# tangjiapeng/DiffuScene

Hardware: AMD Instinct MI355X
Metric: denoiser steps/sec (train + 1000-step sample) at B=256, N=80 objects (higher is better)
Workload: dtype f32 (operands split 3xbf16, 6 products, f32 accumulate); 1 GPU; uncond living/dining rooms (config/uncond/diffusion_livingrooms_instancond_lat32_v.yaml scaled to N=80), B=256 scenes per GPU, N=80, C=65, T=1000, mode=both; global_batch=256, parallelism=single

## Files before the change

### diffuscene_amd/_lib.py

```python
import ctypes as C
import os

_HERE = os.path.dirname(os.path.abspath(__file__))
LIB_PATH = os.path.join(_HERE, "libdiffuscene_hip.so")
if os.environ.get("DSC_HIP_LIB"):
    LIB_PATH = os.path.abspath(os.environ["DSC_HIP_LIB"])

ACT_NONE, ACT_GELU, ACT_SILU, ACT_LEAKY01 = 0, 1, 2, 3
SS_NONE, SS_PER_TOKEN, SS_PER_SCENE, SS_PER_SLOT, SS_BY_INDEX = 0, 1, 2, 3, 4
MEAN_EPS, MEAN_X0, MEAN_V = 0, 1, 2
TILE_GN_80_W8, TILE_GN_80_W4, TILE_160x256, TILE_160x128_W4 = 1, 2, 5, 8
TILE_WAVE_GN, TILE_WAVE_DENSE, TILE_WAVE_GN_64 = 10, 11, 12
F32_TILE_160x256, F32_TILE_160x128, F32_TILE_128x128, F32_TILE_96x128, F32_TILE_64x64 = 0, 1, 2, 3, 4
DSC_PLANES_NONE = -100
GEMM_ROW_INVARIANT = 1
WS_MAX = 64
MAX_TOKENS_PER_SCENE = 160
STATS_MAX_OBJECTS, STATS_ONE_WAVE_MAX = 160, 32

_ERR = {-1: "DSC_EINVAL (bad shape / null pointer)", -2: "DSC_EALIGN (16-byte alignment required)",
        -3: "DSC_ERANGE (size outside kernel limits)"}

c_f32p = C.c_void_p
c_i64p = C.c_void_p
# ... 63 lines not shown

class ColsumItem(C.Structure):
    _fields_ = [("x", C.c_void_p), ("ldx", C.c_int64), ("m", C.c_int32), ("n", C.c_int32), ("out", C.c_void_p)]


class WsBwdItem(C.Structure):
    _fields_ = [("w", C.c_void_p), ("dw_std", C.c_void_p), ("dw", C.c_void_p), ("rows", C.c_int32), ("cols", C.c_int32)]


SIGNATURES = {
    "dsc_version": (C.c_int, []),
    "dsc_gemm_f32": (C.c_int, [C.POINTER(GemmArgs), C.c_void_p]),
    "dsc_gemm_gn_silu_f32": (C.c_int, [C.POINTER(GemmArgs), C.c_void_p]),
    "dsc_split_bf16x3_f32": (C.c_int, [C.POINTER(SplitItem), C.c_int32, C.c_void_p]),
    "dsc_gemm_arithmetic": (C.c_int, [C.POINTER(GemmArgs), C.c_int32]),
    "dsc_gemm_split_tile": (C.c_int, [C.POINTER(GemmArgs), C.c_int32]),
    "dsc_gemm_f32_tile": (C.c_int, [C.POINTER(GemmArgs)]),
    "dsc_gemm_planes_layout": (C.c_int, [C.POINTER(GemmArgs), C.c_int32]),
    "dsc_get_split_wave": (C.c_int, []),
    "dsc_set_split_wave": (C.c_int, [C.c_int32]),
    "dsc_gemm_skinny": (C.c_int, [C.POINTER(GemmArgs), C.c_int32]),
    "dsc_get_skinny": (C.c_int, []),
    "dsc_set_skinny": (C.c_int, [C.c_int32]),
    "dsc_get_gemm_arithmetic": (C.c_int, []),
    "dsc_set_gemm_arithmetic": (C.c_int, [C.c_int32]),
    "dsc_gemm_layernorm_f32": (C.c_int, [C.POINTER(GemmArgs), C.c_void_p]),
    "dsc_gemm_splitk_f32": (C.c_int, [C.POINTER(GemmArgs), C.c_int32, c_f32p, C.c_int64, C.c_void_p]),
    "dsc_linear_smallk_f32": (C.c_int, [c_f32p, C.c_int64, C.c_int32, c_f32p, C.c_int64, c_f32p, c_f32p, C.c_int64,
                                        C.c_int32, C.c_int32, C.c_int32, C.c_void_p]),
    "dsc_linear_smallk_grouped_f32": (C.c_int, [C.POINTER(SmallKItem), C.c_int32, C.c_int32, C.c_int32, C.c_int32, C.c_void_p]),
    "dsc_gather_columns_f32": (C.c_int, [c_f32p, C.c_int64, c_f32p, C.c_int64, C.c_int32, C.POINTER(ColSpan), C.c_int32, C.c_void_p]),
    "dsc_weight_standardize_f32": (C.c_int, [C.POINTER(WsItem), C.c_int32, C.c_float, C.c_void_p]),
    "dsc_layernorm_f32": (C.c_int, [c_f32p, C.c_int64, c_f32p, c_f32p, C.c_int64, c_f32p, C.c_int64, C.c_int32,
                                    C.c_int32, C.c_float, C.c_void_p]),
    "dsc_linear_attention_f32": (C.c_int, [c_f32p, C.c_int64, c_f32p, C.c_int64, c_f32p, C.c_int64, c_f32p, C.c_int64,
                                           C.c_int32, C.c_int32, C.c_int32, C.c_float, C.c_void_p]),
    "dsc_attention_f32": (C.c_int, [c_f32p, C.c_int64, c_f32p, C.c_int64, c_f32p, C.c_int64, c_f32p, C.c_int64,
                                    C.c_int32, C.c_int32, C.c_float, C.c_void_p]),
    "dsc_time_embedding_f32": (C.c_int, [c_i64p, C.c_int32, C.c_int32, c_f32p, C.c_int32, c_f32p, c_f32p, C.c_void_p]),
    "dsc_activation_f32": (C.c_int, [c_f32p, c_f32p, C.c_int64, C.c_int32, C.c_void_p]),
    "dsc_q_sample_f32": (C.c_int, [c_f32p, c_f32p, c_i64p, c_f32p, c_f32p, c_f32p, c_f32p, C.c_int32, C.c_int64, C.c_int32,
                                   C.c_void_p]),
    "dsc_p_sample_f32": (C.c_int, [c_f32p, c_f32p, c_f32p, c_i64p, c_f32p, c_f32p, c_f32p, c_f32p, c_f32p, c_f32p,
                                   c_f32p, C.c_int32, C.c_int32, C.c_int32, C.c_int64, C.c_int32, C.c_void_p]),
    "dsc_device_error_count": (C.c_int64, [C.c_int32]),
    "dsc_add_scalar_i64": (C.c_int, [c_i64p, C.c_int32, C.c_int64, C.c_void_p]),
# ... 174 lines not shown
```

### diffuscene_amd/csrc/blocks.hip

```cpp
#include "dsc_common.h"

namespace {

struct WsBatch { dsc_ws_item it[DSC_WS_MAX]; };

__device__ __forceinline__ float block_sum_256(float v, float* red) {
    v = wave_sum(v);
    const int lane = threadIdx.x & 63, wave = threadIdx.x >> 6;
    __syncthreads();
    if (lane == 0) red[wave] = v;
    __syncthreads();
    return red[0] + red[1] + red[2] + red[3];
}

__global__ __launch_bounds__(256) void ws_kernel(const WsBatch b, const float eps) {
    __shared__ float red[4];
    const dsc_ws_item it = b.it[blockIdx.y];
    const int row = blockIdx.x;
    if (row >= it.rows) return;
    const float* w = it.w + (int64_t)row * it.cols;
    float* o = it.out + (int64_t)row * it.cols;
    constexpr int MAXE = 8;
    float v[MAXE];
    float s = 0.f;
// ... 40 lines not shown
    }
    const float var = wave_sum(s2) * (1.0f / 512.0f);
    const float rs = 1.0f / sqrtf(var + eps);
    const f32x4 ga = *reinterpret_cast<const f32x4*>(g + lane * 4);
    const f32x4 gb = *reinterpret_cast<const f32x4*>(g + 256 + lane * 4);
    f32x4 oa, ob;
#pragma unroll
    for (int e = 0; e < 4; ++e) {
        oa[e] = (a[e] - mean) * rs * ga[e];
        ob[e] = (b[e] - mean) * rs * gb[e];
    }
    if (res) {
        const float* rr = res + (int64_t)row * ldr;
        const f32x4 ra = *reinterpret_cast<const f32x4*>(rr + lane * 4);
        const f32x4 rb = *reinterpret_cast<const f32x4*>(rr + 256 + lane * 4);
#pragma unroll
        for (int e = 0; e < 4; ++e) { oa[e] += ra[e]; ob[e] += rb[e]; }
    }
    float* yr = y + (int64_t)row * ldy;
    *reinterpret_cast<f32x4*>(yr + lane * 4) = oa;
    *reinterpret_cast<f32x4*>(yr + 256 + lane * 4) = ob;
}

constexpr int MAXTOK = 160;
constexpr int HP = 33;
constexpr int LP = 36;

__global__ __launch_bounds__(256) void linear_attention_kernel(const float* __restrict__ q, int64_t ldq,
                                                               const float* __restrict__ k, int64_t ldk,
                                                               const float* __restrict__ v, int64_t ldv,
                                                               float* __restrict__ out, int64_t ldo,
                                                               int nq, int nk, float scale) {
    extern __shared__ __attribute__((aligned(16))) float lds[];
    float* Ks = lds;
    float* Vs = Ks + nk * LP;
    float* Qs = Vs + nk * LP;
    float* ctx = Qs + nq * LP;
    const int b = blockIdx.x >> 2, h = blockIdx.x & 3;
    const int tid = threadIdx.x;
    const float* kb = k + (int64_t)b * nk * ldk + h * 32;
    const float* vb = v + (int64_t)b * nk * ldv + h * 32;
    const float* qb = q + (int64_t)b * nq * ldq + h * 32;
    for (int f = tid; f < nk * 8; f += 256) {
        const int j = f >> 3, c4 = (f & 7) * 4;
        *reinterpret_cast<f32x4*>(Ks + j * LP + c4) = *reinterpret_cast<const f32x4*>(kb + (int64_t)j * ldk + c4);
        *reinterpret_cast<f32x4*>(Vs + j * LP + c4) = *reinterpret_cast<const f32x4*>(vb + (int64_t)j * ldv + c4);
    }
    for (int f = tid; f < nq * 8; f += 256) {
        const int i = f >> 3, c4 = (f & 7) * 4;
// ... 60 lines not shown
#pragma unroll
            for (int e = 0; e < 4; ++e) { a[e] = qv[e] * inv; c[e] = qv[4 + e] * inv; }
            *reinterpret_cast<f32x4*>(Qs + i * LP + part * 8) = a;
            *reinterpret_cast<f32x4*>(Qs + i * LP + part * 8 + 4) = c;
        }
        __builtin_amdgcn_wave_barrier();
        if (ok) {
            f32x4 o0 = {0.f, 0.f, 0.f, 0.f}, o1 = {0.f, 0.f, 0.f, 0.f};
#pragma unroll 8
            for (int d = 0; d < 32; ++d) {
                const float qd = Qs[i * LP + d];
                const f32x4 c0 = *reinterpret_cast<const f32x4*>(ctx + d * LP + part * 8);
                const f32x4 c1 = *reinterpret_cast<const f32x4*>(ctx + d * LP + part * 8 + 4);
#pragma unroll
                for (int e = 0; e < 4; ++e) { o0[e] += c0[e] * qd; o1[e] += c1[e] * qd; }
            }
            float* orow = out + ((int64_t)b * nq + i) * ldo + h * 32 + part * 8;
            *reinterpret_cast<f32x4*>(orow) = o0;
            *reinterpret_cast<f32x4*>(orow + 4) = o1;
        }
    }
}

__global__ __launch_bounds__(512) void attention_kernel(const float* __restrict__ q, int64_t ldq,
                                                        const float* __restrict__ k, int64_t ldk,
                                                        const float* __restrict__ v, int64_t ldv,
                                                        float* __restrict__ out, int64_t ldo, int n, float scale) {
    extern __shared__ __attribute__((aligned(16))) float att_lds[];
    float* Ks = att_lds;
    float* Vs = Ks + n * LP;
    const int b = blockIdx.x >> 2, h = blockIdx.x & 3;
    const int tid = threadIdx.x;
    const float* kb = k + (int64_t)b * n * ldk + h * 32;
    const float* vb = v + (int64_t)b * n * ldv + h * 32;
    const int nthr = blockDim.x, rows = nthr >> 2;
    for (int f = tid; f < n * 8; f += nthr) {
        const int j = f >> 3, c4 = (f & 7) * 4;
        *reinterpret_cast<f32x4*>(Ks + j * LP + c4) = *reinterpret_cast<const f32x4*>(kb + (int64_t)j * ldk + c4);
        *reinterpret_cast<f32x4*>(Vs + j * LP + c4) = *reinterpret_cast<const f32x4*>(vb + (int64_t)j * ldv + c4);
    }
    __syncthreads();
    const int part = tid & 3;
    for (int i0 = 0; i0 < n; i0 += rows) {
        const int i = i0 + (tid >> 2);
        const bool ok = i < n;
        const float* qr = q + ((int64_t)b * n + (ok ? i : 0)) * ldq + h * 32 + part * 8;
// ... 147 lines not shown
        if (items[i].cols > 2048) return DSC_ERANGE;
        b.it[i] = items[i];
        if (items[i].rows > maxrows) maxrows = items[i].rows;
    }
    DSC_CLEAR_STALE_ERROR();
    hipLaunchKernelGGL(ws_kernel, dim3(maxrows, count), dim3(256), 0, static_cast<hipStream_t>(stream), b, eps);
    DSC_LAUNCH_CHECK();
    return 0;
}

extern "C" int dsc_layernorm_f32(const float* x, int64_t ldx, const float* g, const float* residual, int64_t ldr,
                                 float* y, int64_t ldy, int32_t m, int32_t d, float eps, dsc_stream_t stream) {
    if (!x || !g || !y || m < 1) return DSC_EINVAL;
    if (d != 512) return DSC_ERANGE;
    if (!dsc_aligned16(x) || !dsc_aligned16(g) || !dsc_aligned16(y) || (ldx & 3) || (ldy & 3)) return DSC_EALIGN;
    if (residual && (!dsc_aligned16(residual) || (ldr & 3))) return DSC_EALIGN;
    DSC_CLEAR_STALE_ERROR();
    hipLaunchKernelGGL(layernorm512_kernel, dim3((m + 3) / 4), dim3(256), 0, static_cast<hipStream_t>(stream),
                       x, ldx, g, residual, ldr, y, ldy, m, eps);
    DSC_LAUNCH_CHECK();
    return 0;
}

extern "C" int dsc_linear_attention_f32(const float* q, int64_t ldq, const float* k, int64_t ldk,
                                        const float* v, int64_t ldv, float* out, int64_t ldo,
                                        int32_t scenes, int32_t nq, int32_t nk, float scale, dsc_stream_t stream) {
    if (!q || !k || !v || !out || scenes < 1 || nq < 1 || nk < 1) return DSC_EINVAL;
    if (nk > MAXTOK) return DSC_ERANGE;
    if (!dsc_aligned16(q) || !dsc_aligned16(k) || !dsc_aligned16(v) || !dsc_aligned16(out) ||
        (ldq & 3) || (ldk & 3) || (ldv & 3) || (ldo & 3)) return DSC_EALIGN;
    if (nq > MAXTOK) return DSC_ERANGE;
    const size_t lds = sizeof(float) * ((size_t)(2 * nk + nq) * LP + 32 * LP);
    static bool attr_set = false;
    if (!attr_set) {
        hipError_t e = hipFuncSetAttribute(reinterpret_cast<const void*>(linear_attention_kernel),
                                           hipFuncAttributeMaxDynamicSharedMemorySize, 96 * 1024);
        if (e != hipSuccess) return (int)e;
        attr_set = true;
    }
    DSC_CLEAR_STALE_ERROR();
    hipLaunchKernelGGL(linear_attention_kernel, dim3(scenes * DSC_HEADS), dim3(256), lds,
                       static_cast<hipStream_t>(stream), q, ldq, k, ldk, v, ldv, out, ldo, nq, nk, scale);
    DSC_LAUNCH_CHECK();
    return 0;
}

extern "C" int dsc_attention_f32(const float* q, int64_t ldq, const float* k, int64_t ldk,
                                 const float* v, int64_t ldv, float* out, int64_t ldo,
                                 int32_t scenes, int32_t n, float scale, dsc_stream_t stream) {
    if (!q || !k || !v || !out || scenes < 1 || n < 1) return DSC_EINVAL;
    if (n > MAXTOK) return DSC_ERANGE;
    if (!dsc_aligned16(q) || !dsc_aligned16(k) || !dsc_aligned16(v) || !dsc_aligned16(out) ||
        (ldq & 3) || (ldk & 3) || (ldv & 3) || (ldo & 3)) return DSC_EALIGN;
    DSC_CLEAR_STALE_ERROR();
// ... 75 lines not shown
```

### diffuscene_amd/csrc/dsc_common.h

```cpp
#pragma once
#include <hip/hip_runtime.h>
#include <stdint.h>
#include <type_traits>
#include "../../include/diffuscene_hip.h"

typedef float f32x2 __attribute__((ext_vector_type(2)));
typedef float f32x4 __attribute__((ext_vector_type(4)));
typedef float f32x16 __attribute__((ext_vector_type(16)));

#define DSC_WAVE 64

#include <utility>
template <class F, int... I>
__device__ __forceinline__ void dsc_static_for_impl(F&& f, std::integer_sequence<int, I...>) { (f(std::integral_constant<int, I>{}), ...); }
template <int N, class F>
__device__ __forceinline__ void dsc_static_for(F&& f) { dsc_static_for_impl(f, std::make_integer_sequence<int, N>{}); }

#define DSC_CLEAR_STALE_ERROR() ((void)hipGetLastError())

#define DSC_LAUNCH_CHECK()                                   \
    do {                                                     \
        hipError_t e__ = hipGetLastError();                  \
        if (e__ != hipSuccess) return (int)e__;              \
    } while (0)
// ... 25 lines not shown
        const float t = __builtin_amdgcn_rcpf(fmaf(0.3275911f, a, 1.0f));
        float p = fmaf(1.061405429f, t, -1.453152027f);
        p = fmaf(p, t, 1.421413741f);
        p = fmaf(p, t, -0.284496736f);
        p = fmaf(p, t, 0.254829592f);
        const float e = __expf(-a * a);
        const float cdf = 0.5f * (1.0f + copysignf(1.0f - p * t * e, xv));
        return fmaf(xv * 0.39894228040143267794f, e, cdf);
    }
    if (act == DSC_ACT_SILU) {
        const float sig = __builtin_amdgcn_rcpf(1.0f + __expf(-xv));
        return sig * fmaf(xv, 1.0f - sig, 1.0f);
    }
    if (act == DSC_ACT_LEAKY01) return xv > 0.0f ? 1.0f : 0.1f;
    return 1.0f;
}

static inline unsigned dsc_attention_threads(int n) {
    if (n <= 64) return 256;
    const int waves = (n + 15) / 16;
    return waves >= 8 ? 512u : 64u * (unsigned)waves;
}

__device__ __forceinline__ float wave_sum(float v) {
#pragma unroll
    for (int o = 32; o > 0; o >>= 1) v += __shfl_xor(v, o, 64);
    return v;
}
__device__ __forceinline__ float wave_sum_dpp(float v) {
    auto dpp_add = [](float x, auto ctrl, auto row_mask, auto bank_mask) {
        const int y = __builtin_amdgcn_update_dpp(0, __builtin_bit_cast(int, x), decltype(ctrl)::value, decltype(row_mask)::value,
                                                  decltype(bank_mask)::value, true);
        return x + __builtin_bit_cast(float, y);
    };
    using std::integral_constant;
    v = dpp_add(v, integral_constant<int, 0x111>{}, integral_constant<int, 0xf>{}, integral_constant<int, 0xf>{});
    v = dpp_add(v, integral_constant<int, 0x112>{}, integral_constant<int, 0xf>{}, integral_constant<int, 0xf>{});
    v = dpp_add(v, integral_constant<int, 0x114>{}, integral_constant<int, 0xf>{}, integral_constant<int, 0xf>{});
    v = dpp_add(v, integral_constant<int, 0x118>{}, integral_constant<int, 0xf>{}, integral_constant<int, 0xf>{});
    v = dpp_add(v, integral_constant<int, 0x142>{}, integral_constant<int, 0xa>{}, integral_constant<int, 0xf>{});
    v = dpp_add(v, integral_constant<int, 0x143>{}, integral_constant<int, 0xc>{}, integral_constant<int, 0xf>{});
    return __builtin_bit_cast(float, __builtin_amdgcn_readlane(__builtin_bit_cast(int, v), 63));
}
__device__ __forceinline__ float wave_max(float v) {
#pragma unroll
    for (int o = 32; o > 0; o >>= 1) v = fmaxf(v, __shfl_xor(v, o, 64));
// ... 34 lines not shown
```

### diffuscene_amd/csrc/train.hip

```cpp
#define DSC_BAD_INDEX_COUNTER
#include "dsc_common.h"

namespace {

constexpr int TN_BK = 32;
constexpr int TN_LD = 132;

struct TnArgs {
    const float* a1; long lda1; int k1;
    const float* a2; long lda2; int k2;
    const float* dy; long ldd;
    float* out; long ldo;
    float* bias_out;
    long slab;
    long bias_slab;
    int m, n, kvalid;
    int chunk;
    int ktiles;
};

__device__ __forceinline__ void tn_block(const TnArgs& p, const int it, const int jt, const int split, float* As, float* Bs) {
    const int tid = threadIdx.x, lane = tid & 63, wave = tid >> 6;
    const int wi = wave >> 1, wj = wave & 1;
    const int l31 = lane & 31, half = lane >> 5;
// ... 769 lines not shown
        const float m2 = wave_sum(t2) * (1.0f / 512.0f);
        f32x4 oa, ob;
#pragma unroll
        for (int e = 0; e < 4; ++e) {
            oa[e] = rs * (ha[e] - m1 - xa[e] * m2);
            ob[e] = rs * (hb[e] - m1 - xb[e] * m2);
        }
        if (addend) {
            const float* ar = addend + row * ldadd;
            oa += *reinterpret_cast<const f32x4*>(ar + lane * 4);
            ob += *reinterpret_cast<const f32x4*>(ar + 256 + lane * 4);
        }
        float* o = dx + row * lddx;
        *reinterpret_cast<f32x4*>(o + lane * 4) = oa;
        *reinterpret_cast<f32x4*>(o + 256 + lane * 4) = ob;
    }
#pragma unroll
    for (int e = 0; e < 4; ++e) { red[wave][lane * 4 + e] = dga[e]; red[wave][256 + lane * 4 + e] = dgb[e]; }
    __syncthreads();
    for (int c = threadIdx.x; c < 512; c += 256)
        dg_partial[(long)blockIdx.x * 512 + c] = (red[0][c] + red[1][c]) + (red[2][c] + red[3][c]);
}

constexpr int HP = 33;
constexpr int LP = 36;

__global__ __launch_bounds__(256) void linear_attention_bwd_kernel(
        const float* __restrict__ q, long ldq, const float* __restrict__ k, long ldk, const float* __restrict__ v, long ldv,
        const float* __restrict__ dout, long ldo, float* __restrict__ dq, long lddq, float* __restrict__ dk, long lddk,
        float* __restrict__ dv, long lddv, int nq, int nk, float scale) {
    extern __shared__ __attribute__((aligned(16))) float lds[];
    float* Ks = lds;
    float* Vs = Ks + nk * LP;
    float* DK = Vs + nk * LP;
    float* Qs = DK + nk * LP;
    float* DO = Qs + nq * LP;
    float* ctx = DO + nq * LP;
    float* dctx = ctx + 32 * LP;
    float* cvec = dctx + 32 * LP;
    const int b = blockIdx.x >> 2, h = blockIdx.x & 3;
    const int tid = threadIdx.x;
    for (int f = tid; f < nk * 8; f += 256) {
        const int j = f >> 3, c4 = (f & 7) * 4;
        const long row = (long)b * nk + j;
        *reinterpret_cast<f32x4*>(Ks + j * LP + c4) = *reinterpret_cast<const f32x4*>(k + row * ldk + h * 32 + c4);
        *reinterpret_cast<f32x4*>(Vs + j * LP + c4) = *reinterpret_cast<const f32x4*>(v + row * ldv + h * 32 + c4);
    }
    for (int f = tid; f < nq * 8; f += 256) {
// ... 361 lines not shown
        float dkv[8] = {0.f, 0.f, 0.f, 0.f, 0.f, 0.f, 0.f, 0.f}, dvv[8] = {0.f, 0.f, 0.f, 0.f, 0.f, 0.f, 0.f, 0.f};
        for (int i = 0; i < n; ++i) {
            const float pij = P[i * PS + jc], ds = DS[i * PS + jc];
            const f32x4 q0 = *reinterpret_cast<const f32x4*>(Qs + i * LQ + part * 8);
            const f32x4 q1 = *reinterpret_cast<const f32x4*>(Qs + i * LQ + part * 8 + 4);
            const f32x4 d0 = *reinterpret_cast<const f32x4*>(DO + i * LQ + part * 8);
            const f32x4 d1 = *reinterpret_cast<const f32x4*>(DO + i * LQ + part * 8 + 4);
#pragma unroll
            for (int e = 0; e < 4; ++e) {
                dkv[e] += ds * q0[e]; dkv[4 + e] += ds * q1[e];
                dvv[e] += pij * d0[e]; dvv[4 + e] += pij * d1[e];
            }
        }
        if (ok) {
            float* ok_ = dk + ((long)b * n + j) * lddk + h * 32 + part * 8;
            float* ov = dv + ((long)b * n + j) * lddv + h * 32 + part * 8;
            f32x4 a0, a1, b0, b1;
#pragma unroll
            for (int e = 0; e < 4; ++e) { a0[e] = dkv[e]; a1[e] = dkv[4 + e]; b0[e] = dvv[e]; b1[e] = dvv[4 + e]; }
            *reinterpret_cast<f32x4*>(ok_) = a0; *reinterpret_cast<f32x4*>(ok_ + 4) = a1;
            *reinterpret_cast<f32x4*>(ov) = b0; *reinterpret_cast<f32x4*>(ov + 4) = b1;
        }
    }
}

__global__ void act_bwd_kernel(const float* __restrict__ x, const float* __restrict__ dy, float* __restrict__ dx,
                               long count, int act) {
    long i = (long)blockIdx.x * blockDim.x + threadIdx.x;
    const long stride = (long)gridDim.x * blockDim.x;
    for (; i < count; i += stride) {
        dx[i] = dy[i] * dsc_act_grad(x[i], act);
    }
}

__global__ __launch_bounds__(256) void transpose_kernel(const float* __restrict__ in, long ldi, float* __restrict__ out,
                                                       long ldo, int rows, int cols) {
    __shared__ float tile[32][33];
    const int c0 = blockIdx.x * 32, r0 = blockIdx.y * 32;
    const int tx = threadIdx.x & 31, ty = threadIdx.x >> 5;
    for (int r = ty; r < 32; r += 8)
        if (r0 + r < rows && c0 + tx < cols) tile[r][tx] = in[(long)(r0 + r) * ldi + c0 + tx];
    __syncthreads();
    for (int c = ty; c < 32; c += 8)
        if (c0 + c < cols && r0 + tx < rows) out[(long)(c0 + c) * ldo + r0 + tx] = tile[tx][c];
}

// ... 223 lines not shown
extern "C" int dsc_layernorm_bwd_f32(const float* x, int64_t ldx, const float* g, const float* dy, int64_t ldy, float* dx,
                                     int64_t lddx, const float* addend, int64_t ldadd, float* dg_partial, int32_t partial_rows,
                                     int32_t m, int32_t d, float eps, dsc_stream_t stream) {
    if (!x || !g || !dy || !dx || !dg_partial || m < 1 || partial_rows < 1) return DSC_EINVAL;
    if (d != 512) return DSC_ERANGE;
    if (!dsc_aligned16(x) || !dsc_aligned16(g) || !dsc_aligned16(dy) || !dsc_aligned16(dx) || (ldx & 3) || (ldy & 3) ||
        (lddx & 3) || (addend && (!dsc_aligned16(addend) || (ldadd & 3)))) return DSC_EALIGN;
    DSC_CLEAR_STALE_ERROR();
    hipLaunchKernelGGL(layernorm_bwd_kernel, dim3(partial_rows), dim3(256), 0, static_cast<hipStream_t>(stream),
                       x, (long)ldx, g, dy, (long)ldy, dx, (long)lddx, addend, (long)ldadd, dg_partial, m, eps);
    DSC_LAUNCH_CHECK();
    return 0;
}

extern "C" int dsc_linear_attention_bwd_f32(const float* q, int64_t ldq, const float* k, int64_t ldk, const float* v,
                                            int64_t ldv, const float* dout, int64_t ldo, float* dq, int64_t lddq,
                                            float* dk, int64_t lddk, float* dv, int64_t lddv, int32_t scenes, int32_t nq,
                                            int32_t nk, float scale, dsc_stream_t stream) {
    if (!q || !k || !v || !dout || !dq || !dk || !dv || scenes < 1 || nq < 1 || nk < 1) return DSC_EINVAL;
    if (nq > 160 || nk > 160) return DSC_ERANGE;
    if ((ldq | ldk | ldv | ldo | lddq | lddk | lddv) & 3) return DSC_EALIGN;
    if (!dsc_aligned16(q) || !dsc_aligned16(k) || !dsc_aligned16(v) || !dsc_aligned16(dout) || !dsc_aligned16(dq) ||
        !dsc_aligned16(dk) || !dsc_aligned16(dv)) return DSC_EALIGN;
    const size_t lds = sizeof(float) * ((size_t)(3 * nk + 2 * nq) * LP + 2 * 32 * LP + 32);
    static bool attr_set = false;
    if (!attr_set) {
        hipError_t e = hipFuncSetAttribute(reinterpret_cast<const void*>(linear_attention_bwd_kernel),
                                           hipFuncAttributeMaxDynamicSharedMemorySize, 160 * 1024);
        if (e != hipSuccess) return (int)e;
        attr_set = true;
    }
    DSC_CLEAR_STALE_ERROR();
    hipLaunchKernelGGL(linear_attention_bwd_kernel, dim3(scenes * DSC_HEADS), dim3(256), lds,
                       static_cast<hipStream_t>(stream), q, (long)ldq, k, (long)ldk, v, (long)ldv, dout, (long)ldo,
                       dq, (long)lddq, dk, (long)lddk, dv, (long)lddv, nq, nk, scale);
    DSC_LAUNCH_CHECK();
    return 0;
}

extern "C" int dsc_attention_bwd_f32(const float* q, int64_t ldq, const float* k, int64_t ldk, const float* v, int64_t ldv,
                                     const float* dout, int64_t ldo, float* dq, int64_t lddq, float* dk, int64_t lddk,
                                     float* dv, int64_t lddv, int32_t scenes, int32_t n, float scale, dsc_stream_t stream) {
    if (!q || !k || !v || !dout || !dq || !dk || !dv || scenes < 1 || n < 1) return DSC_EINVAL;
    if (n > 160) return DSC_ERANGE;
    if ((ldq | ldk | ldv | ldo | lddq | lddk | lddv) & 3) return DSC_EALIGN;
    if (!dsc_aligned16(q) || !dsc_aligned16(k) || !dsc_aligned16(v) || !dsc_aligned16(dout) || !dsc_aligned16(dq) ||
        !dsc_aligned16(dk) || !dsc_aligned16(dv)) return DSC_EALIGN;
    if (n <= 96) {
        const size_t ldc = sizeof(float) * ((size_t)4 * n * 36 + (size_t)2 * n * (n + 1));
        static bool attr_c = false;
        if (!attr_c) {
            hipError_t e = hipFuncSetAttribute(reinterpret_cast<const void*>(attention_bwd_cached_kernel),
                                               hipFuncAttributeMaxDynamicSharedMemorySize, 160 * 1024);
            if (e != hipSuccess) return (int)e;
            attr_c = true;
        }
        DSC_CLEAR_STALE_ERROR();
        hipLaunchKernelGGL(attention_bwd_cached_kernel, dim3(scenes * DSC_HEADS), dim3(dsc_attention_threads(n)), ldc,
                           static_cast<hipStream_t>(stream), q, (long)ldq, k, (long)ldk, v, (long)ldv, dout, (long)ldo, dq,
                           (long)lddq, dk, (long)lddk, dv, (long)lddv, n, scale);
        DSC_LAUNCH_CHECK();
        return 0;
    }
    const size_t lds = sizeof(float) * ((size_t)4 * n * HP + 3 * n);
    static bool attr_set = false;
    if (!attr_set) {
        hipError_t e = hipFuncSetAttribute(reinterpret_cast<const void*>(attention_bwd_kernel),
                                           hipFuncAttributeMaxDynamicSharedMemorySize, 160 * 1024);
        if (e != hipSuccess) return (int)e;
        attr_set = true;
    }
    DSC_CLEAR_STALE_ERROR();
// ... 331 lines not shown
```

### include/diffuscene_hip.h

```cpp
#ifndef DIFFUSCENE_HIP_H
#define DIFFUSCENE_HIP_H

#include <stdint.h>

#ifdef __cplusplus
extern "C" {
#endif

typedef void* dsc_stream_t;

#define DSC_EINVAL   (-1)
#define DSC_EALIGN   (-2)
#define DSC_ERANGE   (-3)

#define DSC_ACT_NONE 0
#define DSC_ACT_GELU 1
#define DSC_ACT_SILU 2
#define DSC_ACT_LEAKY01 3

#define DSC_SS_NONE      0
#define DSC_SS_PER_TOKEN 1
#define DSC_SS_PER_SCENE 2
#define DSC_SS_PER_SLOT  3
#define DSC_SS_BY_INDEX  4
// ... 88 lines not shown
#define DSC_SMALLK_MAX 4
typedef struct dsc_smallk_item { const float* x; int64_t ldx; int32_t k_in; const float* w; int64_t ldw; const float* bias;
                                 float* y; int64_t ldy; } dsc_smallk_item;
int dsc_linear_smallk_grouped_f32(const dsc_smallk_item* items, int32_t count, int32_t m, int32_t n, int32_t act_out,
                                  dsc_stream_t stream);
typedef struct dsc_col_span { int32_t src_col, dst_col, width; } dsc_col_span;
int dsc_gather_columns_f32(float* dst, int64_t ldd, const float* src, int64_t lds, int32_t rows, const dsc_col_span* spans,
                           int32_t count, dsc_stream_t stream);

#define DSC_WS_MAX 64
typedef struct dsc_ws_item { const float* w; float* out; int32_t rows; int32_t cols; } dsc_ws_item;
int dsc_weight_standardize_f32(const dsc_ws_item* items, int32_t count, float eps, dsc_stream_t stream);

int dsc_layernorm_f32(const float* x, int64_t ldx, const float* g, const float* residual, int64_t ldr,
                      float* y, int64_t ldy, int32_t m, int32_t d, float eps, dsc_stream_t stream);

int dsc_linear_attention_f32(const float* q, int64_t ldq, const float* k, int64_t ldk,
                             const float* v, int64_t ldv, float* out, int64_t ldo,
                             int32_t scenes, int32_t nq, int32_t nk, float scale, dsc_stream_t stream);

int dsc_attention_f32(const float* q, int64_t ldq, const float* k, int64_t ldk,
                      const float* v, int64_t ldv, float* out, int64_t ldo,
                      int32_t scenes, int32_t n, float scale, dsc_stream_t stream);

int dsc_time_embedding_f32(const int64_t* t, int32_t b, int32_t dim, const float* table, int32_t table_rows,
                           const float* freq, float* out, dsc_stream_t stream);

int dsc_activation_f32(const float* x, float* y, int64_t count, int32_t act, dsc_stream_t stream);


int64_t dsc_device_error_count(int32_t reset);

int dsc_q_sample_f32(const float* x0, const float* noise, const int64_t* t,
                     const float* sqrt_ac, const float* sqrt_1mac,
                     float* x_t, float* v_out, int32_t b, int64_t inner, int32_t num_timesteps, dsc_stream_t stream);

#define DSC_MEAN_EPS 0
#define DSC_MEAN_X0  1
#define DSC_MEAN_V   2
int dsc_p_sample_f32(const float* x_t, const float* model_out, const float* noise, const int64_t* t,
                     const float* ca, const float* cb, const float* coef1, const float* coef2,
                     const float* sigma, float* out, float* x0_out ,
                     int32_t mean_type, int32_t clip, int32_t b, int64_t inner, int32_t num_timesteps,
                     dsc_stream_t stream);

int dsc_add_scalar_i64(int64_t* t, int32_t count, int64_t delta, dsc_stream_t stream);
// ... 218 lines not shown
```

Baseline: 62.66 steps/s.

## Add MFMA-based linear and softmax attention kernels for forward and backward

Adds new linear-attention forward/backward kernels and a softmax-attention backward kernel (n<=96) that compute the key-value context and output products with 16x16x4 f32 MFMA instructions instead of scalar FMA loops. Token counts are padded to multiples of 16 and the kernels are enabled by default through a DSC_ATTN_CORES toggle. The aim is to cut the compute time of the attention stages. The costs are extra LDS padding, larger thread blocks, and different f32 accumulation order, since full-f32 MFMA is used rather than the split-bf16 path.

```diff
diff --git a/diffuscene_amd/_lib.py b/diffuscene_amd/_lib.py
--- a/diffuscene_amd/_lib.py
+++ b/diffuscene_amd/_lib.py
@@ -109,6 +109,8 @@
     "dsc_gemm_skinny": (C.c_int, [C.POINTER(GemmArgs), C.c_int32]),
     "dsc_get_skinny": (C.c_int, []),
     "dsc_set_skinny": (C.c_int, [C.c_int32]),
+    "dsc_get_attention_cores": (C.c_int, []),
+    "dsc_set_attention_cores": (C.c_int, [C.c_int32]),
     "dsc_get_gemm_arithmetic": (C.c_int, []),
     "dsc_set_gemm_arithmetic": (C.c_int, [C.c_int32]),
     "dsc_gemm_layernorm_f32": (C.c_int, [C.POINTER(GemmArgs), C.c_void_p]),
diff --git a/diffuscene_amd/csrc/blocks.hip b/diffuscene_amd/csrc/blocks.hip
--- a/diffuscene_amd/csrc/blocks.hip
+++ b/diffuscene_amd/csrc/blocks.hip
@@ -1,4 +1,5 @@
 #include "dsc_common.h"
+#include <cstdlib>
 
 namespace {
 
@@ -86,9 +87,8 @@
     *reinterpret_cast<f32x4*>(yr + 256 + lane * 4) = ob;
 }
 
-constexpr int MAXTOK = 160;
-constexpr int HP = 33;
-constexpr int LP = 36;
+constexpr int MAXTOK = DSC_ATT_MAXTOK;
+constexpr int LP = DSC_ATT_LP;
 
 __global__ __launch_bounds__(256) void linear_attention_kernel(const float* __restrict__ q, int64_t ldq,
                                                                const float* __restrict__ k, int64_t ldk,
@@ -195,6 +195,127 @@
     }
 }
 
+__global__ __launch_bounds__(640) void linear_attention_mfma_kernel(const float* __restrict__ q, int64_t ldq,
+                                                                    const float* __restrict__ k, int64_t ldk,
+                                                                    const float* __restrict__ v, int64_t ldv,
+                                                                    float* __restrict__ out, int64_t ldo,
+                                                                    int nq, int nk, float scale) {
+    extern __shared__ __attribute__((aligned(16))) float lds_m[];
+    const int npq = (nq + 15) & ~15, npk = (nk + 15) & ~15;
+    float* Ks = lds_m;
+    float* Vs = Ks + npk * LP;
+    float* Qs = Vs + npk * LP;
+    float* ctx = Qs + npq * LP;
+    const int b = blockIdx.x >> 2, h = blockIdx.x & 3;
+    const int tid = threadIdx.x, nthr = blockDim.x, lane = tid & 63, wave = tid >> 6, nwaves = nthr >> 6;
+    const int l15 = lane & 15, g = lane >> 4;
+    const float* kb = k + (int64_t)b * nk * ldk + h * 32;
+    const float* vb = v + (int64_t)b * nk * ldv + h * 32;
+    const float* qb = q + (int64_t)b * nq * ldq + h * 32;
+    const f32x4 zero4 = {0.f, 0.f, 0.f, 0.f};
+    for (int f = tid; f < npk * 8; f += nthr) {
+        const int j = f >> 3, c4 = (f & 7) * 4;
+        f32x4 kv = zero4, vv = zero4;
+        if (j < nk) {
+            kv = *reinterpret_cast<const f32x4*>(kb + (int64_t)j * ldk + c4);
+            vv = *reinterpret_cast<const f32x4*>(vb + (int64_t)j * ldv + c4);
+        }
+        *reinterpret_cast<f32x4*>(Ks + j * LP + c4) = kv;
+        *reinterpret_cast<f32x4*>(Vs + j * LP + c4) = vv;
+    }
+    for (int f = tid; f < npq * 8; f += nthr) {
+        const int i = f >> 3, c4 = (f & 7) * 4;
+        f32x4 qv = zero4;
+        if (i < nq) qv = *reinterpret_cast<const f32x4*>(qb + (int64_t)i * ldq + c4);
+        *reinterpret_cast<f32x4*>(Qs + i * LP + c4) = qv;
+    }
+    __syncthreads();
+    if (tid < 256) {
+        const int d = tid >> 3, part = tid & 7;
+        float mx = -INFINITY;
+        for (int j = part; j < nk; j += 8) mx = fmaxf(mx, Ks[j * LP + d]);
+        mx = fmaxf(mx, __shfl_xor(mx, 1, 64));
+        mx = fmaxf(mx, __shfl_xor(mx, 2, 64));
+        mx = fmaxf(mx, __shfl_xor(mx, 4, 64));
+        float sm = 0.f;
+        for (int j = part; j < nk; j += 8) {
+            const float e = expf(Ks[j * LP + d] - mx);
+            Ks[j * LP + d] = e;
+            sm += e;
+        }
+        sm += __shfl_xor(sm, 1, 64);
+        sm += __shfl_xor(sm, 2, 64);
+        sm += __shfl_xor(sm, 4, 64);
+        const float inv = 1.0f / sm;
+        for (int j = part; j < nk; j += 8) Ks[j * LP + d] *= inv;
+    }
+    for (int i0 = 0; i0 < nq; i0 += (nthr >> 2)) {
+        const int i = i0 + (tid >> 2), part = tid & 3;
+        const bool ok = i < nq;
+        float qv[8];
+        float mx = -INFINITY;
+        if (ok) {
+            const f32x4 a = *reinterpret_cast<const f32x4*>(Qs + i * LP + part * 8);
+            const f32x4 c = *reinterpret_cast<const f32x4*>(Qs + i * LP + part * 8 + 4);
+#pragma unroll
+            for (int e = 0; e < 4; ++e) { qv[e] = a[e]; qv[4 + e] = c[e]; }
+#pragma unroll
+            for (int e = 0; e < 8; ++e) mx = fmaxf(mx, qv[e]);
+        }
+        mx = fmaxf(mx, __shfl_xor(mx, 1, 64));
+        mx = fmaxf(mx, __shfl_xor(mx, 2, 64));
+        float sm = 0.f;
+        if (ok) {
+#pragma unroll
+            for (int e = 0; e < 8; ++e) { qv[e] = expf(qv[e] - mx); sm += qv[e]; }
+        }
+        sm += __shfl_xor(sm, 1, 64);
+        sm += __shfl_xor(sm, 2, 64);
+        if (ok) {
+            const float inv = scale / sm;
+            f32x4 a, c;
+#pragma unroll
+            for (int e = 0; e < 4; ++e) { a[e] = qv[e] * inv; c[e] = qv[4 + e] * inv; }
+            *reinterpret_cast<f32x4*>(Qs + i * LP + part * 8) = a;
+            *reinterpret_cast<f32x4*>(Qs + i * LP + part * 8 + 4) = c;
+        }
+    }
+    __syncthreads();
+    for (int t = wave; t < 4; t += nwaves) {
+        const int d0 = (t >> 1) * 16, e0 = (t & 1) * 16;
+        f32x4 acc = zero4;
+        for (int j0 = 0; j0 < npk; j0 += 4)
+            acc = dsc_mma16(Ks[(j0 + g) * LP + d0 + l15], Vs[(j0 + g) * LP + e0 + l15], acc);
+#pragma unroll
+        for (int r = 0; r < 4; ++r) ctx[(d0 + 4 * g + r) * LP + e0 + l15] = acc[r];
+    }
+    __syncthreads();
+    for (int ib = wave; ib * 16 < npq; ib += nwaves) {
+        const int i0 = ib * 16;
+        float qf[8];
+#pragma unroll
+        for (int s = 0; s < 8; ++s) qf[s] = Qs[(i0 + l15) * LP + 4 * s + g];
+        f32x4 o0 = zero4, o1 = zero4;
+#pragma unroll
+        for (int s = 0; s < 8; ++s) {
+            o0 = dsc_mma16(qf[s], ctx[(4 * s + g) * LP + l15], o0);
+            o1 = dsc_mma16(qf[s], ctx[(4 * s + g) * LP + 16 + l15], o1);
+        }
+#pragma unroll
+        for (int r = 0; r < 4; ++r) {
+            Qs[(i0 + 4 * g + r) * LP + l15] = o0[r];
+            Qs[(i0 + 4 * g + r) * LP + 16 + l15] = o1[r];
+        }
+        __builtin_amdgcn_wave_barrier();
+#pragma unroll
+        for (int f = lane; f < 128; f += 64) {
+            const int i = i0 + (f >> 3), c4 = (f & 7) * 4;
+            if (i < nq)
+                *reinterpret_cast<f32x4*>(out + ((int64_t)b * nq + i) * ldo + h * 32 + c4) = *reinterpret_cast<const f32x4*>(Qs + i * LP + c4);
+        }
+    }
+}
+
 __global__ __launch_bounds__(512) void attention_kernel(const float* __restrict__ q, int64_t ldq,
                                                         const float* __restrict__ k, int64_t ldk,
                                                         const float* __restrict__ v, int64_t ldv,
@@ -388,6 +509,17 @@
     return 0;
 }
 
+static int g_attn_cores = -1;
+int dsc_attention_cores_enabled() {
+    if (g_attn_cores < 0) {
+        const char* e = std::getenv("DSC_ATTN_CORES");
+        g_attn_cores = (e && e[0] == '0') ? 0 : 1;
+    }
+    return g_attn_cores;
+}
+extern "C" int dsc_get_attention_cores(void) { return dsc_attention_cores_enabled(); }
+extern "C" int dsc_set_attention_cores(int32_t on) { const int prev = dsc_attention_cores_enabled(); g_attn_cores = on ? 1 : 0; return prev; }
+
 extern "C" int dsc_linear_attention_f32(const float* q, int64_t ldq, const float* k, int64_t ldk,
                                         const float* v, int64_t ldv, float* out, int64_t ldo,
                                         int32_t scenes, int32_t nq, int32_t nk, float scale, dsc_stream_t stream) {
@@ -396,6 +528,17 @@
     if (!dsc_aligned16(q) || !dsc_aligned16(k) || !dsc_aligned16(v) || !dsc_aligned16(out) ||
         (ldq & 3) || (ldk & 3) || (ldv & 3) || (ldo & 3)) return DSC_EALIGN;
     if (nq > MAXTOK) return DSC_ERANGE;
+    {
+        const int npq = dsc_att_pad16(nq), npk = dsc_att_pad16(nk);
+        const size_t ldm = sizeof(float) * ((size_t)(2 * npk + npq) * LP + 32 * LP);
+        if (dsc_attention_cores_enabled() && ldm <= 64 * 1024) {
+            DSC_CLEAR_STALE_ERROR();
+            hipLaunchKernelGGL(linear_attention_mfma_kernel, dim3(scenes * DSC_HEADS), dim3(dsc_att_mfma_threads(nq > nk ? nq : nk)), ldm,
+                               static_cast<hipStream_t>(stream), q, ldq, k, ldk, v, ldv, out, ldo, nq, nk, scale);
+            DSC_LAUNCH_CHECK();
+            return 0;
+        }
+    }
     const size_t lds = sizeof(float) * ((size_t)(2 * nk + nq) * LP + 32 * LP);
     static bool attr_set = false;
     if (!attr_set) {
diff --git a/diffuscene_amd/csrc/dsc_common.h b/diffuscene_amd/csrc/dsc_common.h
--- a/diffuscene_amd/csrc/dsc_common.h
+++ b/diffuscene_amd/csrc/dsc_common.h
@@ -71,6 +71,18 @@
     return waves >= 8 ? 512u : 64u * (unsigned)waves;
 }
 
+constexpr int DSC_ATT_MAXTOK = 160;
+constexpr int DSC_ATT_HP = 33;
+constexpr int DSC_ATT_LP = 36;
+
+static inline int dsc_att_pad16(int n) { return (n + 15) & ~15; }
+static inline unsigned dsc_att_mfma_threads(int n) {
+    const int waves = (n + 15) / 16;
+    return 64u * (unsigned)(waves < 4 ? 4 : waves);
+}
+int dsc_attention_cores_enabled();
+__device__ __forceinline__ f32x4 dsc_mma16(float a, float b, f32x4 acc) { return __builtin_amdgcn_mfma_f32_16x16x4f32(a, b, acc, 0, 0, 0); }
+
 __device__ __forceinline__ float wave_sum(float v) {
 #pragma unroll
     for (int o = 32; o > 0; o >>= 1) v += __shfl_xor(v, o, 64);
diff --git a/diffuscene_amd/csrc/train.hip b/diffuscene_amd/csrc/train.hip
--- a/diffuscene_amd/csrc/train.hip
+++ b/diffuscene_amd/csrc/train.hip
@@ -815,8 +815,8 @@
         dg_partial[(long)blockIdx.x * 512 + c] = (red[0][c] + red[1][c]) + (red[2][c] + red[3][c]);
 }
 
-constexpr int HP = 33;
-constexpr int LP = 36;
+constexpr int HP = DSC_ATT_HP;
+constexpr int LP = DSC_ATT_LP;
 
 __global__ __launch_bounds__(256) void linear_attention_bwd_kernel(
         const float* __restrict__ q, long ldq, const float* __restrict__ k, long ldk, const float* __restrict__ v, long ldv,
@@ -1224,6 +1224,373 @@
             *reinterpret_cast<f32x4*>(ov) = b0; *reinterpret_cast<f32x4*>(ov + 4) = b1;
         }
     }
+}
+
+__device__ __forceinline__ void att_store_rows16(const float* rows_lds, float* __restrict__ dst, long ld, int tok0, int ntok, int lane) {
+#pragma unroll
+    for (int f = lane; f < 128; f += 64) {
+        const int t = tok0 + (f >> 3), c4 = (f & 7) * 4;
+        if (t < ntok) *reinterpret_cast<f32x4*>(dst + (long)t * ld + c4) = *reinterpret_cast<const f32x4*>(rows_lds + t * LP + c4);
+    }
+}
+
+__global__ __launch_bounds__(640) void linear_attention_bwd_mfma_kernel(
+        const float* __restrict__ q, long ldq, const float* __restrict__ k, long ldk, const float* __restrict__ v, long ldv,
+        const float* __restrict__ dout, long ldo, float* __restrict__ dq, long lddq, float* __restrict__ dk, long lddk,
+        float* __restrict__ dv, long lddv, int nq, int nk, float scale) {
+    extern __shared__ __attribute__((aligned(16))) float lds[];
+    const int npq = (nq + 15) & ~15, npk = (nk + 15) & ~15;
+    float* Ks = lds;
+    float* Vs = Ks + npk * LP;
+    float* Qs = Vs + npk * LP;
+    float* DO = Qs + npq * LP;
+    float* ctx = DO + npq * LP;
+    float* dctx = ctx + 32 * LP;
+    float* cvec = dctx + 32 * LP;
+    const int b = blockIdx.x >> 2, h = blockIdx.x & 3;
+    const int tid = threadIdx.x, nthr = blockDim.x, lane = tid & 63, wave = tid >> 6, nwaves = nthr >> 6;
+    const int l15 = lane & 15, g = lane >> 4;
+    const f32x4 zero4 = {0.f, 0.f, 0.f, 0.f};
+    for (int f = tid; f < npk * 8; f += nthr) {
+        const int j = f >> 3, c4 = (f & 7) * 4;
+        const long row = (long)b * nk + j;
+        f32x4 kv = zero4, vv = zero4;
+        if (j < nk) {
+            kv = *reinterpret_cast<const f32x4*>(k + row * ldk + h * 32 + c4);
+            vv = *reinterpret_cast<const f32x4*>(v + row * ldv + h * 32 + c4);
+        }
+        *reinterpret_cast<f32x4*>(Ks + j * LP + c4) = kv;
+        *reinterpret_cast<f32x4*>(Vs + j * LP + c4) = vv;
+    }
+    for (int f = tid; f < npq * 8; f += nthr) {
+        const int i = f >> 3, c4 = (f & 7) * 4;
+        const long row = (long)b * nq + i;
+        f32x4 qv = zero4, dv4 = zero4;
+        if (i < nq) {
+            qv = *reinterpret_cast<const f32x4*>(q + row * ldq + h * 32 + c4);
+            dv4 = *reinterpret_cast<const f32x4*>(dout + row * ldo + h * 32 + c4);
+        }
+        *reinterpret_cast<f32x4*>(Qs + i * LP + c4) = qv;
+        *reinterpret_cast<f32x4*>(DO + i * LP + c4) = dv4;
+    }
+    __syncthreads();
+    if (tid < 256) {
+        const int d = tid >> 3, part = tid & 7;
+        float mx = -INFINITY;
+        for (int j = part; j < nk; j += 8) mx = fmaxf(mx, Ks[j * LP + d]);
+        mx = fmaxf(mx, __shfl_xor(mx, 1, 64));
+        mx = fmaxf(mx, __shfl_xor(mx, 2, 64));
+        mx = fmaxf(mx, __shfl_xor(mx, 4, 64));
+        float sm = 0.f;
+        for (int j = part; j < nk; j += 8) { const float e = expf(Ks[j * LP + d] - mx); Ks[j * LP + d] = e; sm += e; }
+        sm += __shfl_xor(sm, 1, 64);
+        sm += __shfl_xor(sm, 2, 64);
+        sm += __shfl_xor(sm, 4, 64);
+        const float inv = 1.0f / sm;
+        for (int j = part; j < nk; j += 8) Ks[j * LP + d] *= inv;
+    }
+    for (int i0 = 0; i0 < nq; i0 += (nthr >> 2)) {
+        const int i = i0 + (tid >> 2), part = tid & 3;
+        const bool ok = i < nq;
+        float qv[8];
+        float mx = -INFINITY;
+        if (ok) {
+            const f32x4 a = *reinterpret_cast<const f32x4*>(Qs + i * LP + part * 8);
+            const f32x4 c = *reinterpret_cast<const f32x4*>(Qs + i * LP + part * 8 + 4);
+#pragma unroll
+            for (int e = 0; e < 4; ++e) { qv[e] = a[e]; qv[4 + e] = c[e]; }
+#pragma unroll
+            for (int e = 0; e < 8; ++e) mx = fmaxf(mx, qv[e]);
+        }
+        mx = fmaxf(mx, __shfl_xor(mx, 1, 64));
+        mx = fmaxf(mx, __shfl_xor(mx, 2, 64));
+        float sm = 0.f;
+        if (ok) {
+#pragma unroll
+            for (int e = 0; e < 8; ++e) { qv[e] = expf(qv[e] - mx); sm += qv[e]; }
+        }
+        sm += __shfl_xor(sm, 1, 64);
+        sm += __shfl_xor(sm, 2, 64);
+        if (ok) {
+            const float inv = scale / sm;
+            f32x4 a, c;
+#pragma unroll
+            for (int e = 0; e < 4; ++e) { a[e] = qv[e] * inv; c[e] = qv[4 + e] * inv; }
+            *reinterpret_cast<f32x4*>(Qs + i * LP + part * 8) = a;
+            *reinterpret_cast<f32x4*>(Qs + i * LP + part * 8 + 4) = c;
+        }
+    }
+    __syncthreads();
+    for (int t = wave; t < 8; t += nwaves) {
+        const int d0 = ((t >> 1) & 1) * 16, e0 = (t & 1) * 16;
+        const float* A = t < 4 ? Ks : Qs;
+        const float* B = t < 4 ? Vs : DO;
+        const int np = t < 4 ? npk : npq;
+        f32x4 acc = zero4;
+        for (int j0 = 0; j0 < np; j0 += 4) acc = dsc_mma16(A[(j0 + g) * LP + d0 + l15], B[(j0 + g) * LP + e0 + l15], acc);
+        float* C = t < 4 ? ctx : dctx;
+#pragma unroll
+        for (int r = 0; r < 4; ++r) C[(d0 + 4 * g + r) * LP + e0 + l15] = acc[r];
+    }
+    __syncthreads();
+    if (wave * 16 < npq) {
+        const int i0 = wave * 16;
+        float df[8];
+#pragma unroll
+        for (int s = 0; s < 8; ++s) df[s] = DO[(i0 + l15) * LP + 4 * s + g];
+        f32x4 a0 = zero4, a1 = zero4;
+#pragma unroll
+        for (int s = 0; s < 8; ++s) {
+            a0 = dsc_mma16(df[s], ctx[l15 * LP + 4 * s + g], a0);
+            a1 = dsc_mma16(df[s], ctx[(16 + l15) * LP + 4 * s + g], a1);
+        }
+#pragma unroll
+        for (int r = 0; r < 4; ++r) {
+            DO[(i0 + 4 * g + r) * LP + l15] = a0[r];
+            DO[(i0 + 4 * g + r) * LP + 16 + l15] = a1[r];
+        }
+        __builtin_amdgcn_wave_barrier();
+        const int i = i0 + (lane >> 2), part = lane & 3;
+        const f32x4 d0 = *reinterpret_cast<const f32x4*>(DO + i * LP + part * 8), d1 = *reinterpret_cast<const f32x4*>(DO + i * LP + part * 8 + 4);
+        const f32x4 s0 = *reinterpret_cast<const f32x4*>(Qs + i * LP + part * 8), s1 = *reinterpret_cast<const f32x4*>(Qs + i * LP + part * 8 + 4);
+        double dot = 0.0;
+#pragma unroll
+        for (int e = 0; e < 4; ++e) dot += (double)d0[e] * (double)s0[e];
+#pragma unroll
+        for (int e = 0; e < 4; ++e) dot += (double)d1[e] * (double)s1[e];
+        dot += __shfl_xor(dot, 1, 64);
+        dot += __shfl_xor(dot, 2, 64);
+        if (i < nq) {
+            const float corr = (float)(dot / (double)scale);
+            f32x4 a, c;
+#pragma unroll
+            for (int e = 0; e < 4; ++e) { a[e] = s0[e] * (d0[e] - corr); c[e] = s1[e] * (d1[e] - corr); }
+            float* o = dq + ((long)b * nq + i) * lddq + h * 32 + part * 8;
+            *reinterpret_cast<f32x4*>(o) = a;
+            *reinterpret_cast<f32x4*>(o + 4) = c;
+        }
+    }
+    f32x4 v0 = zero4, v1 = zero4;
+    const int j0 = wave * 16;
+    if (j0 < npk) {
+        float vf[8], kf[8];
+#pragma unroll
+        for (int s = 0; s < 8; ++s) { vf[s] = Vs[(j0 + l15) * LP + 4 * s + g]; kf[s] = Ks[(j0 + l15) * LP + 4 * s + g]; }
+        f32x4 k0 = zero4, k1 = zero4;
+#pragma unroll
+        for (int s = 0; s < 8; ++s) {
+            k0 = dsc_mma16(vf[s], dctx[l15 * LP + 4 * s + g], k0);
+            k1 = dsc_mma16(vf[s], dctx[(16 + l15) * LP + 4 * s + g], k1);
+            v0 = dsc_mma16(kf[s], dctx[(4 * s + g) * LP + l15], v0);
+            v1 = dsc_mma16(kf[s], dctx[(4 * s + g) * LP + 16 + l15], v1);
+        }
+#pragma unroll
+        for (int r = 0; r < 4; ++r) {
+            Vs[(j0 + 4 * g + r) * LP + l15] = k0[r];
+            Vs[(j0 + 4 * g + r) * LP + 16 + l15] = k1[r];
+        }
+    }
+    __syncthreads();
+    if (tid < 256) {
+        const int d = tid >> 3, part = tid & 7;
+        float sdd = 0.f;
+        for (int j = part; j < nk; j += 8) sdd += Vs[j * LP + d] * Ks[j * LP + d];
+        sdd += __shfl_xor(sdd, 1, 64);
+        sdd += __shfl_xor(sdd, 2, 64);
+        sdd += __shfl_xor(sdd, 4, 64);
+        if (part == 0) cvec[d] = sdd;
+    }
+    __syncthreads();
+    if (j0 < npk) {
+#pragma unroll
+        for (int f = lane; f < 128; f += 64) {
+            const int j = j0 + (f >> 3), c4 = (f & 7) * 4;
+            if (j < nk) {
+                const f32x4 ks4 = *reinterpret_cast<const f32x4*>(Ks + j * LP + c4);
+                const f32x4 dk4 = *reinterpret_cast<const f32x4*>(Vs + j * LP + c4);
+                f32x4 t4;
+#pragma unroll
+                for (int e = 0; e < 4; ++e) t4[e] = ks4[e] * (dk4[e] - cvec[c4 + e]);
+                *reinterpret_cast<f32x4*>(dk + ((long)b * nk + j) * lddk + h * 32 + c4) = t4;
+            }
+        }
+        __builtin_amdgcn_wave_barrier();
+#pragma unroll
+        for (int r = 0; r < 4; ++r) {
+            Ks[(j0 + 4 * g + r) * LP + l15] = v0[r];
+            Ks[(j0 + 4 * g + r) * LP + 16 + l15] = v1[r];
+        }
+        __builtin_amdgcn_wave_barrier();
+        att_store_rows16(Ks, dv + (long)b * nk * lddv + h * 32, lddv, j0, nk, lane);
+    }
+}
+
+template <int NT>
+__global__ __launch_bounds__(NT < 4 ? 256 : 64 * NT) void attention_bwd_mfma_kernel(
+        const float* __restrict__ q, long ldq, const float* __restrict__ k, long ldk, const float* __restrict__ v, long ldv,
+        const float* __restrict__ dout, long ldo, float* __restrict__ dq, long lddq, float* __restrict__ dk, long lddk,
+        float* __restrict__ dv, long lddv, int n, float scale) {
+    extern __shared__ __attribute__((aligned(16))) float lds[];
+    constexpr int NP = 16 * NT;
+    float* Qs = lds;
+    float* Ks = Qs + NP * LP;
+    float* Vs = Ks + NP * LP;
+    float* DO = Vs + NP * LP;
+    float* rmx = DO + NP * LP;
+    float* rinv = rmx + NP;
+    float* rD = rinv + NP;
+    const int b = blockIdx.x >> 2, h = blockIdx.x & 3;
+    const int tid = threadIdx.x, nthr = blockDim.x, lane = tid & 63, wave = tid >> 6;
+    const int l15 = lane & 15, g = lane >> 4;
+    const int lperm = 4 * (l15 & 3) + (l15 >> 2);
+    const f32x4 zero4 = {0.f, 0.f, 0.f, 0.f};
+    for (int f = tid; f < NP * 8; f += nthr) {
+        const int j = f >> 3, c4 = (f & 7) * 4;
+        const long row = (long)b * n + j;
+        f32x4 qv = zero4, kv = zero4, vv = zero4, dv4 = zero4;
+        if (j < n) {
+            qv = *reinterpret_cast<const f32x4*>(q + row * ldq + h * 32 + c4);
+            kv = *reinterpret_cast<const f32x4*>(k + row * ldk + h * 32 + c4);
+            vv = *reinterpret_cast<const f32x4*>(v + row * ldv + h * 32 + c4);
+            dv4 = *reinterpret_cast<const f32x4*>(dout + row * ldo + h * 32 + c4);
+        }
+#pragma unroll
+        for (int e = 0; e < 4; ++e) qv[e] *= scale;
+        *reinterpret_cast<f32x4*>(Qs + j * LP + c4) = qv;
+        *reinterpret_cast<f32x4*>(Ks + j * LP + c4) = kv;
+        *reinterpret_cast<f32x4*>(Vs + j * LP + c4) = vv;
+        *reinterpret_cast<f32x4*>(DO + j * LP + c4) = dv4;
+    }
+    __syncthreads();
+    const int t0 = wave * 16;
+    f32x4 q0 = zero4, q1 = zero4, q0b = zero4, q1b = zero4;
+    if (wave < NT) {
+        float qf[8], of[8];
+#pragma unroll
+        for (int s = 0; s < 8; ++s) { qf[s] = Qs[(t0 + l15) * LP + 4 * s + g]; of[s] = DO[(t0 + l15) * LP + 4 * s + g]; }
+        f32x4 S[NT], dP[NT];
+#pragma unroll
+        for (int t = 0; t < NT; ++t) {
+            f32x4 sp[4], dp[4];
+#pragma unroll
+            for (int p = 0; p < 4; ++p) {
+                sp[p] = zero4; dp[p] = zero4;
+#pragma unroll
+                for (int s = 2 * p; s < 2 * p + 2; ++s) {
+                    sp[p] = dsc_mma16(Ks[(16 * t + lperm) * LP + 4 * s + g], qf[s], sp[p]);
+                    dp[p] = dsc_mma16(Vs[(16 * t + lperm) * LP + 4 * s + g], of[s], dp[p]);
+                }
+            }
+            S[t] = (sp[0] + sp[1]) + (sp[2] + sp[3]);
+            dP[t] = (dp[0] + dp[1]) + (dp[2] + dp[3]);
+        }
+        float mx = -INFINITY;
+#pragma unroll
+        for (int t = 0; t < NT; ++t)
+#pragma unroll
+            for (int r = 0; r < 4; ++r)
+                if (16 * t + 4 * r + g < n) mx = fmaxf(mx, S[t][r]);
+        mx = fmaxf(mx, __shfl_xor(mx, 16, 64));
+        mx = fmaxf(mx, __shfl_xor(mx, 32, 64));
+        double smd = 0.0, Dnd = 0.0;
+#pragma unroll
+        for (int t = 0; t < NT; ++t)
+#pragma unroll
+            for (int r = 0; r < 4; ++r) {
+                const float pj = (16 * t + 4 * r + g < n) ? expf(S[t][r] - mx) : 0.f;
+                S[t][r] = pj;
+                smd += (double)pj;
+                Dnd += (double)pj * (double)dP[t][r];
+            }
+        smd += __shfl_xor(smd, 16, 64);
+        smd += __shfl_xor(smd, 32, 64);
+        Dnd += __shfl_xor(Dnd, 16, 64);
+        Dnd += __shfl_xor(Dnd, 32, 64);
+        const float inv = (float)(1.0 / smd);
+        const float Di = (float)(Dnd / smd);
+        if (g == 0) { rmx[t0 + l15] = mx; rinv[t0 + l15] = inv; rD[t0 + l15] = Di; }
+#pragma unroll
+        for (int t = 0; t < NT; ++t)
+#pragma unroll
+            for (int r = 0; r < 4; ++r) {
+                const float ds = (16 * t + 4 * r + g < n) ? (S[t][r] * inv) * (dP[t][r] - Di) : 0.f;
+                if (t & 1) {
+                    q0b = dsc_mma16(ds, Ks[(16 * t + 4 * r + g) * LP + l15], q0b);
+                    q1b = dsc_mma16(ds, Ks[(16 * t + 4 * r + g) * LP + 16 + l15], q1b);
+                } else {
+                    q0 = dsc_mma16(ds, Ks[(16 * t + 4 * r + g) * LP + l15], q0);
+                    q1 = dsc_mma16(ds, Ks[(16 * t + 4 * r + g) * LP + 16 + l15], q1);
+                }
+            }
+        q0 += q0b; q1 += q1b;
+    }
+    __syncthreads();
+    f32x4 k0 = zero4, k1 = zero4, v0 = zero4, v1 = zero4, k0b = zero4, k1b = zero4, v0b = zero4, v1b = zero4;
+    if (wave < NT) {
+        float kf[8], vf[8];
+#pragma unroll
+        for (int s = 0; s < 8; ++s) { kf[s] = Ks[(t0 + l15) * LP + 4 * s + g]; vf[s] = Vs[(t0 + l15) * LP + 4 * s + g]; }
+        const bool key_ok = t0 + l15 < n;
+#pragma unroll
+        for (int t = 0; t < NT; ++t) {
+            f32x4 sp[4], dp[4];
+#pragma unroll
+            for (int p = 0; p < 4; ++p) {
+                sp[p] = zero4; dp[p] = zero4;
+#pragma unroll
+                for (int s = 2 * p; s < 2 * p + 2; ++s) {
+                    sp[p] = dsc_mma16(Qs[(16 * t + lperm) * LP + 4 * s + g], kf[s], sp[p]);
+                    dp[p] = dsc_mma16(DO[(16 * t + lperm) * LP + 4 * s + g], vf[s], dp[p]);
+                }
+            }
+            const f32x4 S = (sp[0] + sp[1]) + (sp[2] + sp[3]);
+            const f32x4 dP = (dp[0] + dp[1]) + (dp[2] + dp[3]);
+#pragma unroll
+            for (int r = 0; r < 4; ++r) {
+                const int i = 16 * t + 4 * r + g;
+                const bool ok = key_ok && i < n;
+                const float pij = ok ? expf(S[r] - rmx[i]) * rinv[i] : 0.f;
+                const float ds = ok ? pij * (dP[r] - rD[i]) : 0.f;
+                if (t & 1) {
+                    v0b = dsc_mma16(pij, DO[i * LP + l15], v0b);
+                    v1b = dsc_mma16(pij, DO[i * LP + 16 + l15], v1b);
+                    k0b = dsc_mma16(ds, Qs[i * LP + l15], k0b);
+                    k1b = dsc_mma16(ds, Qs[i * LP + 16 + l15], k1b);
+                } else {
+                    v0 = dsc_mma16(pij, DO[i * LP + l15], v0);
+                    v1 = dsc_mma16(pij, DO[i * LP + 16 + l15], v1);
+                    k0 = dsc_mma16(ds, Qs[i * LP + l15], k0);
+                    k1 = dsc_mma16(ds, Qs[i * LP + 16 + l15], k1);
+                }
+            }
+        }
+        k0 += k0b; k1 += k1b; v0 += v0b; v1 += v1b;
+    }
+    __syncthreads();
+    if (wave < NT) {
+#pragma unroll
+        for (int r = 0; r < 4; ++r) {
+            const int t = t0 + 4 * g + r;
+            Qs[t * LP + l15] = q0[r] * scale; Qs[t * LP + 16 + l15] = q1[r] * scale;
+            Ks[t * LP + l15] = k0[r]; Ks[t * LP + 16 + l15] = k1[r];
+            Vs[t * LP + l15] = v0[r]; Vs[t * LP + 16 + l15] = v1[r];
+        }
+        __builtin_amdgcn_wave_barrier();
+        att_store_rows16(Qs, dq + (long)b * n * lddq + h * 32, lddq, t0, n, lane);
+        att_store_rows16(Ks, dk + (long)b * n * lddk + h * 32, lddk, t0, n, lane);
+        att_store_rows16(Vs, dv + (long)b * n * lddv + h * 32, lddv, t0, n, lane);
+    }
+}
+
+template <int NT>
+int launch_attention_bwd_mfma(hipStream_t s, int scenes, const float* q, long ldq, const float* k, long ldk, const float* v, long ldv,
+                              const float* dout, long ldo, float* dq, long lddq, float* dk, long lddk, float* dv, long lddv, int n, float scale) {
+    const size_t lds = sizeof(float) * ((size_t)4 * 16 * NT * LP + 3 * 16 * NT);
+    DSC_CLEAR_STALE_ERROR();
+    hipLaunchKernelGGL(attention_bwd_mfma_kernel<NT>, dim3(scenes * DSC_HEADS), dim3(NT < 4 ? 256 : 64 * NT), lds, s,
+                       q, ldq, k, ldk, v, ldv, dout, ldo, dq, lddq, dk, lddk, dv, lddv, n, scale);
+    DSC_LAUNCH_CHECK();
+    return 0;
 }
 
 __global__ void act_bwd_kernel(const float* __restrict__ x, const float* __restrict__ dy, float* __restrict__ dx,
@@ -1493,6 +1860,18 @@
     if ((ldq | ldk | ldv | ldo | lddq | lddk | lddv) & 3) return DSC_EALIGN;
     if (!dsc_aligned16(q) || !dsc_aligned16(k) || !dsc_aligned16(v) || !dsc_aligned16(dout) || !dsc_aligned16(dq) ||
         !dsc_aligned16(dk) || !dsc_aligned16(dv)) return DSC_EALIGN;
+    {
+        const int npq = dsc_att_pad16(nq), npk = dsc_att_pad16(nk);
+        const size_t ldm = sizeof(float) * ((size_t)(2 * npk + 2 * npq) * LP + 2 * 32 * LP + 32);
+        if (dsc_attention_cores_enabled() && ldm <= 64 * 1024) {
+            DSC_CLEAR_STALE_ERROR();
+            hipLaunchKernelGGL(linear_attention_bwd_mfma_kernel, dim3(scenes * DSC_HEADS), dim3(dsc_att_mfma_threads(nq > nk ? nq : nk)), ldm,
+                               static_cast<hipStream_t>(stream), q, (long)ldq, k, (long)ldk, v, (long)ldv, dout, (long)ldo,
+                               dq, (long)lddq, dk, (long)lddk, dv, (long)lddv, nq, nk, scale);
+            DSC_LAUNCH_CHECK();
+            return 0;
+        }
+    }
     const size_t lds = sizeof(float) * ((size_t)(3 * nk + 2 * nq) * LP + 2 * 32 * LP + 32);
     static bool attr_set = false;
     if (!attr_set) {
@@ -1517,8 +1896,18 @@
     if ((ldq | ldk | ldv | ldo | lddq | lddk | lddv) & 3) return DSC_EALIGN;
     if (!dsc_aligned16(q) || !dsc_aligned16(k) || !dsc_aligned16(v) || !dsc_aligned16(dout) || !dsc_aligned16(dq) ||
         !dsc_aligned16(dk) || !dsc_aligned16(dv)) return DSC_EALIGN;
+    if (n <= 96 && dsc_attention_cores_enabled()) {
+        hipStream_t s = static_cast<hipStream_t>(stream);
+#define DSC_ATT_BWD_CASE(NT)                                                                                                        \
+        case NT: return launch_attention_bwd_mfma<NT>(s, scenes, q, (long)ldq, k, (long)ldk, v, (long)ldv, dout, (long)ldo, dq,     \
+                                                      (long)lddq, dk, (long)lddk, dv, (long)lddv, n, scale);
+        switch ((n + 15) / 16) {
+            DSC_ATT_BWD_CASE(1) DSC_ATT_BWD_CASE(2) DSC_ATT_BWD_CASE(3) DSC_ATT_BWD_CASE(4) DSC_ATT_BWD_CASE(5) DSC_ATT_BWD_CASE(6)
+        }
+#undef DSC_ATT_BWD_CASE
+    }
     if (n <= 96) {
-        const size_t ldc = sizeof(float) * ((size_t)4 * n * 36 + (size_t)2 * n * (n + 1));
+        const size_t ldc =sizeof(float) * ((size_t)4 * n * 36 + (size_t)2 * n * (n + 1));
         static bool attr_c = false;
         if (!attr_c) {
             hipError_t e = hipFuncSetAttribute(reinterpret_cast<const void*>(attention_bwd_cached_kernel),
diff --git a/include/diffuscene_hip.h b/include/diffuscene_hip.h
--- a/include/diffuscene_hip.h
+++ b/include/diffuscene_hip.h
@@ -134,6 +134,9 @@
 int dsc_attention_f32(const float* q, int64_t ldq, const float* k, int64_t ldk,
                       const float* v, int64_t ldv, float* out, int64_t ldo,
                       int32_t scenes, int32_t n, float scale, dsc_stream_t stream);
+
+int dsc_get_attention_cores(void);
+int dsc_set_attention_cores(int32_t on);
 
 int dsc_time_embedding_f32(const int64_t* t, int32_t b, int32_t dim, const float* table, int32_t table_rows,
                            const float* freq, float* out, dsc_stream_t stream);
```

After: 63.22 steps/s, median of 6. Within noise of the previous version (+0.9%).
